# sstadick/gzp

Hardware: AMD Instinct MI355X
Metric: BGZF compress MiB/s at level 1, 550 MiB text (higher is better)
Workload: dtype u8; 1 GPU; Single MI355X: 64 KiB BGZF blocks, level 1, 550 MiB text slab, bit-exact vs libdeflate; slab_bytes=576716800, block_size=65280, blocks=8835, level=1, format=bgzf, parallelism=block-shard x1, device=AMD Radeon Graphics (gfx950:sramecc+:xnack-, 256 CUs)

## Files before the change

gzp_amd/csrc/gzpx_kernels.hip:

```cpp
#include <hip/hip_runtime.h>
#include <type_traits>
#include <cstring>

#include "gzpx_device.h"

#ifdef GZPX_EXPERIMENT
#define GZPX_EXP(cfg, bit) (((cfg).debug >> (bit)) & 1u)
#else
#define GZPX_EXP(cfg, bit) 0u
#endif

namespace gzpx {


__device__ __forceinline__ void wave_sync() {
    __builtin_amdgcn_fence(__ATOMIC_SEQ_CST, "wavefront");
    __builtin_amdgcn_wave_barrier();
    __builtin_amdgcn_fence(__ATOMIC_SEQ_CST, "wavefront");
}

__device__ __forceinline__ uint32_t rdlane(uint32_t v, uint32_t l) {
    return (uint32_t)__builtin_amdgcn_readlane((int)v, (int)l);
}
__device__ __forceinline__ uint32_t uniform(uint32_t v) { return (uint32_t)__builtin_amdgcn_readfirstlane((int)v); }

#if defined(__HIP_DEVICE_COMPILE__)
#define GZPX_PIN_VGPR(x) asm volatile("" : "+v"(x))
#else
#define GZPX_PIN_VGPR(x) ((void)0)
#endif

__device__ __forceinline__ uint32_t lz_hash15(uint32_t v) { return (v * 0x1E35A7BDu) >> 17; }

__device__ __forceinline__ uint32_t load_le32_global(const uint8_t *p) {
    const uintptr_t a = (uintptr_t)p;
    const uint32_t *w = (const uint32_t *)(a & ~(uintptr_t)3);
    return __builtin_amdgcn_alignbyte(w[1], w[0], (uint32_t)(a & 3));
}

__device__ __forceinline__ uint32_t wave_reduce_add(uint32_t v) {
    for (int m = 32; m >= 1; m >>= 1) v += __shfl_xor(v, m);
    return v;
}

__device__ __forceinline__ uint32_t wave_inclusive_scan(uint32_t v, unsigned lane) {
    for (int d = 1; d < 64; d <<= 1) {
        uint32_t t = __shfl_up(v, d);
        if (lane >= (unsigned)d) v += t;
    }
    return v;
}

template <int CTRL, int ROW_MASK>
__device__ __forceinline__ uint32_t dpp_zero(uint32_t v) {
    return (uint32_t)__builtin_amdgcn_update_dpp(0, (int)v, CTRL, ROW_MASK, 0xf, false);
}
__device__ __forceinline__ uint32_t wave_incl_add(uint32_t v) {
    v += dpp_zero<0x111, 0xf>(v);
    v += dpp_zero<0x112, 0xf>(v);
    v += dpp_zero<0x114, 0xf>(v);
    v += dpp_zero<0x118, 0xf>(v);
    v += dpp_zero<0x142, 0xa>(v);
    v += dpp_zero<0x143, 0xc>(v);
    return v;
}
__device__ __forceinline__ uint32_t umax32(uint32_t a, uint32_t b) { return a > b ? a : b; }
__device__ __forceinline__ uint32_t wave_incl_max(uint32_t v) {
    v = umax32(v, dpp_zero<0x111, 0xf>(v));
    v = umax32(v, dpp_zero<0x112, 0xf>(v));
    v = umax32(v, dpp_zero<0x114, 0xf>(v));
    v = umax32(v, dpp_zero<0x118, 0xf>(v));
    v = umax32(v, dpp_zero<0x142, 0xa>(v));
    v = umax32(v, dpp_zero<0x143, 0xc>(v));
    return v;
}

template <unsigned NW>
__device__ __forceinline__ uint32_t block_exclusive_scan(uint32_t v, uint32_t *wsum, uint32_t *total) {
    const unsigned tid = threadIdx.x, lane = tid & 63, wave = tid >> 6;
    const uint32_t inc = wave_incl_add(v);
    __syncthreads();
    if (lane == 63) wsum[wave] = inc;
    __syncthreads();
    const uint32_t mine = lane < NW ? wsum[lane] : 0u;
    const uint32_t winc = wave_incl_add(mine);
    *total = rdlane(winc, NW - 1);
    const uint32_t base = wave ? rdlane(winc, wave - 1) : 0u;
    return base + inc - v;
}

__device__ __forceinline__ uint64_t block_exclusive_scan256(uint64_t v, uint64_t *wsum, uint64_t *total) {
    const unsigned tid = threadIdx.x, lane = tid & 63, wave = tid >> 6;
    uint64_t inc = v;
    for (int d = 1; d < 64; d <<= 1) {
        const uint64_t t = __shfl_up(inc, d);
        if (lane >= (unsigned)d) inc += t;
    }
    __syncthreads();
    if (lane == 63) wsum[wave] = inc;
    __syncthreads();
    uint64_t base = 0, tot = 0;
    for (unsigned w = 0; w < 4; w++) {
        const uint64_t s = wsum[w];
        if (w < wave) base += s;
        tot += s;
    }
    *total = tot;
    return base + inc - v;
}

__device__ __forceinline__ void length_slot(uint32_t len, uint32_t &slot, uint32_t &ebits,
                                            uint32_t &eval) {
    const uint32_t x = len - 3;
    if (x < 8) {
        slot = x;
        ebits = 0;
        eval = 0;
    } else if (x == 255) {
        slot = 28;
        ebits = 0;
        eval = 0;
    } else {
        const uint32_t k = 31 - __clz((int)x);
        ebits = k - 2;
        slot = 4 * k - 4 + ((x >> ebits) & 3);
        eval = x & ((1u << ebits) - 1);
    }
}

__device__ __forceinline__ void offset_slot(uint32_t off, uint32_t &slot, uint32_t &ebits,
                                            uint32_t &eval) {
    const uint32_t d = off - 1;
    if (d < 4) {
        slot = d;
        ebits = 0;
        eval = 0;
    } else {
        const uint32_t k = 31 - __clz((int)d);
        ebits = k - 1;
        slot = 2 * k + ((d >> ebits) & 1);
        eval = d & ((1u << ebits) - 1);
    }
}


__device__ __forceinline__ uint32_t precode_order(uint32_t i) {
    const uint64_t lo = 0x22caa324e804a30ull, hi = 0x3c2e1346cull;
    return i < 12u ? (uint32_t)(lo >> (5u * i)) & 31u : (uint32_t)(hi >> (5u * (i - 12u))) & 31u;
}

__device__ __forceinline__ BlockMeta block_meta_of(const Config &cfg, uint64_t slab_len, uint32_t nb, uint32_t is_last,
                                                   uint32_t b) {
    const uint64_t begin = (uint64_t)b * cfg.block_size;
    uint64_t len = slab_len > begin ? slab_len - begin : 0;
    if (len > cfg.block_size) len = cfg.block_size;
    BlockMeta m;
    m.n = (uint32_t)len;
    m.is_last = (is_last && b == nb - 1) ? 1u : 0u;
    m.ntok = 0;
    m.nsub = 0;
    m.payload_bytes = 0;
    m.framed_bytes = 0;
    m.crc = 0;
    m.status = kStatusOk;
    return m;
}

__global__ void k_init_meta(Config cfg, uint64_t slab_len, uint32_t nb, uint32_t is_last,
                            BlockMeta *meta, uint32_t *redo) {
    const uint32_t b = blockIdx.x * blockDim.x + threadIdx.x;
    if (b == 0 && redo) {
        redo[0] = 0;
        redo[1 + nb] = 0;
    }
    if (b >= nb) return;
    meta[b] = block_meta_of(cfg, slab_len, nb, is_last, b);
}

constexpr uint32_t kBuckets = 1u << 15;
constexpr uint32_t kCandSteps = 16;

__device__ __forceinline__ uint2 cand_fetch(const uint32_t *__restrict__ in32, uint32_t mis,
                                            uint32_t p, uint32_t wmax) {
    const uint32_t w = (p + mis) >> 2;
    uint2 v;
    v.x = in32[w < wmax ? w : wmax];
    v.y = in32[w + 1 < wmax ? w + 1 : wmax];
    return v;
}

constexpr uint32_t kCandWaves = 16;

template <int MODE>
__device__ __forceinline__ bool cand_bucket(uint32_t v, uint32_t p, uint32_t &h) {
    if (MODE == 0) {
        h = p != 0 ? lz_hash15(v) : 0;
        return true;
    } else if (MODE == 1) {
        h = p != 0 ? lz_hash15(v & 0xFFFFFFu) : 0;
        return true;
    } else {
        const uint32_t h16 = p != 0 ? (v * 0x1E35A7BDu) >> 16 : 0;
        h = h16 & 32767u;
        return MODE == 2 ? h16 < 32768u : h16 >= 32768u;
    }
}

template <int MODE>
__device__ __forceinline__ void cand_step_safe(uint32_t *tab, uint32_t mis, uint32_t base,
                                               uint32_t lane, uint32_t n, uint2 raw,
                                               uint16_t *__restrict__ cand) {
    const uint32_t p = base + lane;
    uint32_t h = 0;
    const bool owns = cand_bucket<MODE>(__builtin_amdgcn_alignbyte(raw.y, raw.x, (p + mis) & 3u), p, h);
    const bool valid = owns && p + 5 <= n;
    if (!valid) h = 0;
    uint32_t c0 = tab[h];
    uint64_t same = __ballot(valid);
    for (int bit = 0; bit < 15; bit++) {
        const bool one = (h >> bit) & 1u;
        const uint64_t m = __ballot(one);
        same &= one ? m : ~m;
    }
    const uint64_t below = same & ((1ull << lane) - 1ull);
    const bool is_last_of_group = ((same >> lane) >> 1) == 0;
    if (below) c0 = (base + 63u - (uint32_t)__clzll((long long)below)) & 0xFFFFu;
    wave_sync();
    if (valid && is_last_of_group) tab[h] = p & 0xFFFFu;
    wave_sync();
    uint32_t d0 = (p - c0) & 0xFFFFu;
    if (d0 > 32767u) d0 = 0;
    if (MODE < 2 || valid || (MODE == 2 && p + 5 > n)) cand[p] = (uint16_t)(valid ? d0 : 0u);
}

template <int MODE>
__device__ void cand_block_safe(uint32_t *tab, const uint32_t *in32, uint32_t mis, uint32_t wmax, uint32_t n,
                                uint32_t lane, uint16_t *__restrict__ cand) {
    for (uint32_t i = lane; i < kBuckets; i += 64) tab[i] = 0x8000u;
    wave_sync();
    for (uint32_t base = 0; base < n; base += 64) {
        if (base != 0 && (base & 32767u) == 0) {
            const uint32_t dead = (base + 0x8000u) & 0xFFFFu;
            for (uint32_t i = lane; i < kBuckets; i += 64) {
                const uint32_t e = tab[i];
                const uint32_t a = (base - e) & 0xFFFFu;
                if (a == 0 || a > 32767u) tab[i] = dead;
            }
            wave_sync();
        }
        cand_step_safe<MODE>(tab, mis, base, lane, n, cand_fetch(in32, mis, base + lane, wmax), cand);
    }
}

template <int MODE>
__global__ __launch_bounds__(64 * kCandWaves) void k_candidates(Config cfg,
                                                                 const uint8_t *__restrict__ slab,
                                                                 BlockMeta *__restrict__ meta,
                                                                 uint16_t *__restrict__ cand_all,
                                                                 uint64_t slab_len, uint32_t nb, uint32_t is_last,
                                                                 uint32_t *__restrict__ redo, uint32_t *__restrict__ claim) {
    __shared__ uint32_t tab[kBuckets + 64];
    __shared__ uint32_t turn;
    __shared__ uint32_t bad_any;
    const uint32_t tid = threadIdx.x, lane = tid & 63u, wave = tid >> 6;
    constexpr uint32_t kIterPos = 64 * kCandSteps;
    auto block_len = [&](uint32_t blk) -> uint32_t {
        const uint64_t begin = (uint64_t)blk * cfg.block_size;
        const uint64_t len = slab_len > begin ? slab_len - begin : 0;
        return (uint32_t)(len > cfg.block_size ? cfg.block_size : len);
    };
    if (MODE <= 1) {
        for (uint32_t blk = blockIdx.x + tid * gridDim.x; blk < nb; blk += 64 * kCandWaves * gridDim.x)
            meta[blk] = block_meta_of(cfg, slab_len, nb, is_last, blk);
        if (blockIdx.x == 0 && tid == 0) redo[0] = 0;
        if (blockIdx.x == 0 && tid < 8) claim[tid] = 0;
    }
    for (uint32_t i = tid; i < kBuckets + 64; i += 64 * kCandWaves) tab[i] = 0;
    if (tid == 0) {
        turn = 0;
        bad_any = 0;
    }
    __syncthreads();

    struct Cursor {
        uint32_t b, it, n, n_iters, vbase, ibase;
    };
    auto settle = [&](Cursor &c) -> bool {
        for (;;) {
            if (c.b >= nb) return false;
            c.n = block_len(c.b);
            c.n_iters = c.n > cfg.passthrough ? (c.n + kIterPos - 1) / kIterPos : 0u;
            if (c.it < c.n_iters) return true;
            if (c.n_iters) {
                c.vbase += c.n + 32768u;
                c.ibase += c.n_iters;
// ... 2374 lines not shown
                                cl = l1;
                                co = d1;
                                continue;
                            }
                        }
                        if (lazy2) {
                            uint32_t d2 = t_d2[rr + 1u];
                            const uint32_t l2 = (uint32_t)t_l2[rr + 1u] + 3u;
                            if (d2 & kHcOrphan) d2 = cl >= 5u ? d2 & 0x7FFFu : 0u;
                            if (d2 != 0 && l2 >= cl && 4 * (int)(l2 - cl) + (bsr_cur - (31 - __clz((int)d2))) > 6) {
                                nlit += 2u;
                                cp += 2u;
                                cl = l2;
                                co = d2;
                                continue;
                            }
                        }
                        break;
                    }
                    mlen = cl;
                    moff = co;
                    nrel = cp + cl - pos;
                }
                if (mlen == 0) nrel = lane + 1u;
            }
            exp_lap(1);
            uint64_t reach = 0;
            uint32_t q = 0;
            while (q < 64u) {
                reach |= 1ull << q;
                q = (uint32_t)__builtin_amdgcn_readlane((int)nrel, (int)q);
            }
            const uint32_t exit_rel = q;
            exp_lap(2);
            const bool in_r = (reach >> lane) & 1ull;
            const uint32_t cnt = in_r ? nlit + (mlen ? 1u : 0u) : 0u;
            const uint32_t inc = wave_incl_add(cnt);
            const uint32_t tb = inc - cnt;
            const uint64_t mm = __ballot(in_r && mlen != 0);
            const uint32_t mb = (uint32_t)__popcll(mm & lane_below);
            const bool due = in_r && (p >= max_block_end || nseq + mb >= kHcSeqPerSub ||
                                      (num_new + tb >= 512u && p - sub_start >= kMinBlockLen && n - p >= kMinBlockLen) ||
                                      p >= next_recalc);
            const uint64_t dm_real = __ballot(due);
            const uint64_t dm = dm_real | (__ballot(off_tile) & reach);
            const uint32_t e = dm ? (uint32_t)__ffsll((long long)dm) - 1u : 64u;
            const uint64_t commit = e < 64u ? reach & ((1ull << e) - 1ull) : reach;
            exp_lap(3);
            if ((commit >> lane) & 1ull) {
                const uint32_t o = ti + tb;
                for (uint32_t j = 0; j < nlit; j++) {
                    const uint32_t c = t_in[r + j];
                    tok[o + j] = c;
                    atomicAdd(&L.freq[c], 1u);
                    atomicAdd(&L.nw[((c >> 5) & 6u) | (c & 1u)], 1u);
                }
                if (mlen) {
                    tok[o + nlit] = kTokMatch | (moff << 9) | mlen;
                    atomicAdd(&L.nw[8u + (mlen >= 9u ? 1u : 0u)], 1u);
                }
            }
            const uint32_t done_tok = e < 64u ? (uint32_t)__builtin_amdgcn_readlane((int)tb, (int)e)
                                              : (uint32_t)__builtin_amdgcn_readlane((int)inc, 63);
            ti += done_tok;
            num_new += done_tok;
            nseq += (uint32_t)__popcll(mm & commit);
            pos += e < 64u ? e : exit_rel;
            exp_lap(4);
            if (e == 64u) continue;
            if (!((dm_real >> e) & 1ull)) {
                t0 = 0xFFFFFFFFu;
                here = true;
                continue;
            }
            if (pos >= max_block_end || nseq >= kHcSeqPerSub) break;
            if (num_new >= 512u && pos - sub_start >= kMinBlockLen && n - pos >= kMinBlockLen) {
                __syncthreads();
                const uint32_t o = lane < 10 ? L.obs[lane] : 0u, w = lane < 10 ? L.nw[lane] : 0u;
                const uint32_t expected = o * num_new, actual = w * num_obs;
                const uint32_t total_delta = wave_reduce_add(actual > expected ? actual - expected : expected - actual);
                bool end = false;
                if (num_obs > 0) {
                    const uint32_t blen = pos - sub_start, num_items = num_obs + num_new;
                    uint32_t cutoff = num_new * 200u / 512u * num_obs;
                    if (blen < 10000u && num_items < 8192u)
                        cutoff += (uint32_t)((unsigned long long)cutoff * (8192u - num_items) / 8192u);
                    end = total_delta + (blen / 4096u) * num_obs >= cutoff;
                }
                if (end) break;
                if (lane < 10) {
                    L.obs[lane] = o + w;
                    L.nw[lane] = 0;
                }
                num_obs += num_new;
                num_new = 0;
                continue;
            }
            {
                __syncthreads();
                uint32_t f[4], total = 0;
                for (uint32_t k = 0; k < 4; k++) {
                    f[k] = L.freq[lane + 64u * k];
                    total += f[k];
                }
                total = wave_reduce_add(total);
                const uint32_t cutoff = total >> 10;
                uint32_t num_used = 0;
                for (uint32_t k = 0; k < 4; k++) num_used += (uint32_t)__popcll(__ballot(f[k] > cutoff));
                min_len = hc_choose_min_len(num_used, cfg.hc_depth);
                const uint32_t a = n - next_recalc, bb = pos - sub_start;
                next_recalc += a < bb ? a : bb;
            }
        }
        if (lane == 0) {
            sub[cur_sub].tok_begin = sub_start_tok;
            sub[cur_sub].tok_end = ti;
            sub[cur_sub].byte_begin = sub_start;
            sub[cur_sub].byte_len = pos - sub_start;
            sub[cur_sub].is_final = pos == n ? 1u : 0u;
        }
        cur_sub++;
        if (pos == n) break;
    }
    if (lane == 0) {
        meta->ntok = ti;
        meta->nsub = cur_sub;
    }
#ifdef GZPX_EXPERIMENT
    exp_lap(5);
    if (lane == 0)
        for (uint32_t k = 0; k < 8; k++) atomicAdd(&g_exp_cycles[(b & 1023u) * 8u + k], exp_acc[k]);
#endif
}

__global__ void k_hc_init(uint32_t nb, HcState *hc, uint32_t *pending) {
    const uint32_t b = blockIdx.x * blockDim.x + threadIdx.x;
    if (b == 0) *pending = 0;
    if (b >= nb) return;
    HcState s;
    s.done = 0;
    s.min_len = 0;
    s.resume_pos = 0;
    s.tok_carry = 0;
    s.mat_carry = 0;
    s.cur_sub = 0;
    s.rounds = 0;
    s.pad = 0;
    s.sparse = kHcArraysNone;
    hc[b] = s;
}

constexpr uint32_t kHistCopies = 8;
constexpr uint32_t kHistPad = kHistStride + 1;

__global__ __launch_bounds__(256) void k_hist(Config cfg, const BlockMeta *__restrict__ meta_all,
                                              const SubMeta *__restrict__ sub_all,
                                              const uint32_t *__restrict__ tok_all,
                                              uint32_t *__restrict__ hist_all) {
    __shared__ uint32_t hist[kHistCopies * kHistPad];
    const uint32_t tid = threadIdx.x;
    const uint32_t b = blockIdx.x;
    const BlockMeta *meta = meta_all + b;
    if (meta->n <= cfg.passthrough) return;
    const SubMeta *sub = sub_all + (uint64_t)b * cfg.max_sub;
    const uint32_t *tok = tok_all + (uint64_t)b * cfg.stride;
    const uint32_t nsub = meta->nsub;
    uint32_t *mine = hist + (tid & (kHistCopies - 1u)) * kHistPad;
    for (uint32_t s = 0; s < nsub; s++) {
        for (uint32_t i = tid; i < kHistCopies * kHistPad; i += 256) hist[i] = 0;
        __syncthreads();
        const uint32_t t_end = sub[s].tok_end;
        for (uint32_t t0 = sub[s].tok_begin + tid; t0 < t_end; t0 += 4 * 256) {
            uint32_t tk[4];
#pragma unroll
            for (uint32_t k = 0; k < 4; k++) tk[k] = t0 + k * 256 < t_end ? tok[t0 + k * 256] : 0xFFFFFFFFu;
#pragma unroll
            for (uint32_t k = 0; k < 4; k++) {
                const uint32_t t = tk[k];
                if (t == 0xFFFFFFFFu) continue;
                if (t & kTokMatch) {
                    uint32_t ls, le, lv, os, oe, ov;
                    length_slot(t & 0x1FFu, ls, le, lv);
                    offset_slot((t >> 9) & 0xFFFFu, os, oe, ov);
                    atomicAdd(&mine[257 + ls], 1u);
                    atomicAdd(&mine[kNumLitlen + os], 1u);
                } else {
                    atomicAdd(&mine[t], 1u);
                }
            }
        }
        __syncthreads();
        uint32_t *out = hist_all + ((uint64_t)b * cfg.max_sub + s) * kHistStride;
        for (uint32_t i = tid; i < kHistStride; i += 256) {
            uint32_t sum = 0;
#pragma unroll
            for (uint32_t c = 0; c < kHistCopies; c++) sum += hist[c * kHistPad + i];
            out[i] = sum;
        }
        __syncthreads();
    }
}

struct HuffLds {
    union {
        uint32_t key[kNumLitlen];
        uint32_t nfreq[kNumLitlen];
        uint32_t hdr[kHdrWords];
    };
    union {
        uint32_t sfreq[kNumLitlen];
        struct {
            uint32_t sfreq_low[32];
            uint16_t items[kNumLitlen + kNumOffset];
        };
    };
    union {
        uint32_t freq[kNumLitlen];
        struct {
            uint32_t freq_low[kNumLitlen / 2];
            uint16_t parent[kNumLitlen];
        };
    };
    uint32_t lcw[kNumLitlen];
    uint16_t ssym[kNumLitlen];
    uint8_t depth[kNumLitlen];
    uint8_t lens[kNumLitlen + kNumOffset];
    uint8_t olens[kNumOffset + 2];
    uint8_t plens[32];
    uint32_t ocw[kNumOffset];
    uint32_t pcw[32];
    uint32_t pfreq[32];
    uint32_t len_counts[16];
    uint32_t misc[8];
};
static_assert(sizeof(HuffLds) <= 6400, "HuffLds: 25 workgroups per CU");
static_assert(kHdrWords <= kNumLitlen, "header bits fit region A");


__device__ __forceinline__ uint32_t reg5_get(const uint32_t (&r)[5], uint32_t k) {
    const uint32_t j = k >> 6, l = k & 63u;
    uint32_t v = rdlane(r[0], l);
    const uint32_t v1 = rdlane(r[1], l), v2 = rdlane(r[2], l), v3 = rdlane(r[3], l), v4 = rdlane(r[4], l);
    v = j == 1 ? v1 : v;
    v = j == 2 ? v2 : v;
    v = j == 3 ? v3 : v;
    v = j == 4 ? v4 : v;
    return v;
}

template <uint32_t NCH, uint32_t MAXL>
__device__ void make_code(HuffLds &h, uint32_t num_syms, uint32_t compat, uint8_t *lens, uint32_t *cw, uint32_t lane) {
    constexpr uint32_t max_len = MAXL;
    uint32_t used = 0;
    for (uint32_t base = 0; base < num_syms; base += 64) {
        const uint32_t s = base + lane;
        uint32_t f = 0;
        if (s < num_syms) {
            f = h.freq[s];
            h.key[s] = f ? ((f << 10) | s) : 0xFFFFFFFFu;
            lens[s] = 0;
            cw[s] = 0;
        }
        used += (uint32_t)__popcll(__ballot(f != 0));
    }
    wave_sync();
    if (used < 2) {
        if (used == 0 && compat == 1) return;
        if (lane == 0) {
            uint32_t sym = 0;
            if (used)
                for (uint32_t s = 0; s < num_syms; s++)
                    if (h.freq[s]) sym = s;
            const uint32_t other = sym ? sym : 1;
            lens[0] = 1;
            cw[0] = 0;
            lens[other] = 1;
            cw[other] = 1;
        }
        wave_sync();
        return;
    }
    {
        uint32_t at = 0;
        uint32_t k0 = lane < num_syms ? h.key[lane] : 0xFFFFFFFFu;
        for (uint32_t base = 0; base < num_syms; base += 64) {
            const uint32_t s1 = base + 64 + lane;
            const uint32_t k1 = s1 < num_syms ? h.key[s1] : 0xFFFFFFFFu;
            wave_sync();
            const bool u = k0 != 0xFFFFFFFFu;
            const unsigned long long m = __ballot(u);
            if (u) h.key[at + (uint32_t)__popcll(m & ((1ull << lane) - 1ull))] = k0;
            at += (uint32_t)__popcll(m);
            k0 = k1;
        }
    }
    wave_sync();
    for (uint32_t base = 0; base < used; base += 64) {
        const uint32_t s = base + lane;
        const uint32_t k = s < used ? h.key[s] : 0u;
        uint32_t rank = 0;
        for (uint32_t j = 0; j < used; j++) rank += h.key[j] < k ? 1u : 0u;
        if (s < used) {
            h.sfreq[rank] = k >> 10;
            h.ssym[rank] = (uint16_t)(k & 1023u);
        }
    }
    wave_sync();
    if (lane == 0) {
        const uint32_t last = used - 1;
        uint32_t i = 0, bq = 0, e = 0;
        do {
            uint32_t nf;
            if (i + 1 <= last && (bq == e || h.sfreq[i + 1] <= h.nfreq[bq])) {
                nf = h.sfreq[i] + h.sfreq[i + 1];
                i += 2;
            } else if (bq + 2 <= e && (i > last || h.nfreq[bq + 1] < h.sfreq[i])) {
                nf = h.nfreq[bq] + h.nfreq[bq + 1];
                h.parent[bq] = (uint16_t)e;
                h.parent[bq + 1] = (uint16_t)e;
                bq += 2;
            } else {
                nf = h.sfreq[i] + h.nfreq[bq];
                h.parent[bq] = (uint16_t)e;
                i++;
                bq++;
            }
            h.nfreq[e] = nf;
        } while (++e < last);
    }
    wave_sync();
    {
        const uint32_t last = used - 1, root = last - 1;
        uint32_t par[NCH], dep[NCH];
#pragma unroll
        for (uint32_t k = 0; k < NCH; k++) {
            const uint32_t node = lane + 64 * k;
            par[k] = node < root ? h.parent[node] : 0xFFFFu;
            dep[k] = node == root ? 0u : 0xFFu;
            if (node <= root) h.depth[node] = (uint8_t)dep[k];
        }
// ... 512 lines not shown
    return total;
}

struct CrcDirectLds {
    uint32_t table[4][256];
    uint32_t part[kCrcSmall];
};

__device__ uint32_t crc32_direct(CrcDirectLds &l, const uint8_t *__restrict__ in, uint32_t n, const CrcConsts &cc,
                                 uint32_t tid) {
    constexpr uint32_t T = kCrcSmall, kSegB = 256, kChunk = T * kSegB;
    for (uint32_t i = tid; i < 256; i += T) {
        uint32_t c = i;
        for (int k = 0; k < 8; k++) c = (c >> 1) ^ (0xEDB88320u & (0u - (c & 1u)));
        l.table[0][i] = c;
    }
    __syncthreads();
    for (uint32_t i = tid; i < 256; i += T) {
        const uint32_t t0 = l.table[0][i];
        const uint32_t t1 = (t0 >> 8) ^ l.table[0][t0 & 0xFFu];
        const uint32_t t2 = (t1 >> 8) ^ l.table[0][t1 & 0xFFu];
        const uint32_t t3 = (t2 >> 8) ^ l.table[0][t2 & 0xFFu];
        l.table[1][i] = t1;
        l.table[2][i] = t2;
        l.table[3][i] = t3;
    }
    uint32_t total = 0;
    const uint32_t first_len = n ? ((n - 1) % kChunk) + 1 : 0;
    for (uint32_t cb = 0; cb < n || cb == 0; cb += (cb == 0 ? first_len : kChunk)) {
        const uint32_t clen = n == 0 ? 0 : (cb == 0 ? first_len : kChunk);
        __syncthreads();
        const int32_t seg_end_i = (int32_t)clen - (int32_t)kSegB * (int32_t)(T - 1 - tid);
        uint32_t crc = 0;
        if (seg_end_i > 0) {
            const uint32_t sb = seg_end_i > (int32_t)kSegB ? (uint32_t)seg_end_i - kSegB : 0u;
            const uint32_t len = (uint32_t)seg_end_i - sb;
            const uint8_t *p = in + cb + sb;
            uint32_t c = 0xFFFFFFFFu;
            if (len == kSegB) {
                const uint32_t mis = (uint32_t)((uintptr_t)p & 3u);
                const uint32_t *q = (const uint32_t *)(p - mis);
                const bool at_end = cb + (uint32_t)seg_end_i == n && mis == 0;
                uint32_t carry = q[0];
                for (uint32_t g = 0; g < 2; g++) {
                    dword4 v[8];
#pragma unroll
                    for (uint32_t k = 0; k < 8; k++) {
                        if (g == 1 && k == 7 && at_end) {
                            v[k].x = q[61];
                            v[k].y = q[62];
                            v[k].z = q[63];
                            v[k].w = 0;
                        } else {
                            v[k] = *(const dword4 *)(q + 1 + 32 * g + 4 * k);
                        }
                    }
#pragma unroll
                    for (uint32_t k = 0; k < 8; k++) {
                        const uint32_t w[4] = {__builtin_amdgcn_alignbyte(v[k].x, carry, mis),
                                               __builtin_amdgcn_alignbyte(v[k].y, v[k].x, mis),
                                               __builtin_amdgcn_alignbyte(v[k].z, v[k].y, mis),
                                               __builtin_amdgcn_alignbyte(v[k].w, v[k].z, mis)};
                        carry = v[k].w;
#pragma unroll
                        for (uint32_t j = 0; j < 4; j++) {
                            c ^= w[j];
                            c = l.table[3][c & 0xFFu] ^ l.table[2][(c >> 8) & 0xFFu] ^ l.table[1][(c >> 16) & 0xFFu] ^
                                l.table[0][c >> 24];
                        }
                    }
                }
            } else {
                for (uint32_t i = 0; i < len; i++) c = (c >> 8) ^ l.table[0][(c ^ p[i]) & 0xFFu];
            }
            crc = ~c;
        }
        l.part[tid] = crc;
        __syncthreads();
        for (uint32_t level = 0; level < 8; level++) {
            const uint32_t stride = 1u << level;
            const uint32_t left = 2 * stride * tid;
            uint32_t merged = 0;
            const bool act = left < T;
            if (act) merged = gf2_multmodp(cc.pow64[level + 2], l.part[left]) ^ l.part[left + stride];
            __syncthreads();
            if (act) l.part[left] = merged;
            __syncthreads();
        }
        total = cb == 0 ? l.part[0] : (gf2_multmodp(cc.pow_tile, total) ^ l.part[0]);
        if (n == 0) break;
    }
    return total;
}

__global__ __launch_bounds__(kCrcSmall) void k_crc32(Config cfg, const uint8_t *__restrict__ slab,
                                                     BlockMeta *__restrict__ meta_all, CrcConsts cc) {
    __shared__ CrcDirectLds l;
    const uint32_t b = blockIdx.x;
    const uint32_t total = crc32_direct(l, slab + (uint64_t)b * cfg.block_size, meta_all[b].n, cc, threadIdx.x);
    if (threadIdx.x == 0) meta_all[b].crc = total;
}

constexpr uint32_t kScanThreads = 1024;
__global__ __launch_bounds__(kScanThreads) void k_scan(uint32_t nb, const BlockMeta *__restrict__ meta,
                                                       uint64_t *__restrict__ out_off, uint32_t *__restrict__ sizes,
                                                       const SlabResult *__restrict__ prev,
                                                       SlabResult *__restrict__ result) {
    __shared__ uint64_t wsum[kScanThreads / 64];
    __shared__ uint32_t fail_s;
    const uint32_t tid = threadIdx.x, lane = tid & 63u, wave = tid >> 6;
    if (tid == 0) fail_s = 0xFFFFFFFFu;
    __syncthreads();
    const uint32_t per = (nb + kScanThreads - 1) / kScanThreads;
    const uint32_t i0 = tid * per < nb ? tid * per : nb, i1 = i0 + per < nb ? i0 + per : nb;
    uint64_t mine = 0;
    uint32_t bad = 0xFFFFFFFFu;
#pragma unroll 8
    for (uint32_t i = i0; i < i1; i++) {
        mine += meta[i].framed_bytes;
        if (meta[i].status != kStatusOk && bad == 0xFFFFFFFFu) bad = i;
    }
    if (bad != 0xFFFFFFFFu) atomicMin(&fail_s, bad);
    uint64_t inc = mine;
    for (int d = 1; d < 64; d <<= 1) {
        const uint64_t t = __shfl_up(inc, d);
        if (lane >= (unsigned)d) inc += t;
    }
    if (lane == 63) wsum[wave] = inc;
    __syncthreads();
    uint64_t run = prev ? prev->total : 0;
    uint64_t total = run;
    for (uint32_t w = 0; w < kScanThreads / 64; w++) {
        const uint64_t v = wsum[w];
        if (w < wave) run += v;
        total += v;
    }
    run += inc - mine;
#pragma unroll 8
    for (uint32_t i = i0; i < i1; i++) {
        const uint32_t v = meta[i].framed_bytes;
        sizes[i] = v;
        out_off[i] = run;
        run += v;
    }
    if (tid == 0) {
        const uint32_t f = fail_s;
        out_off[nb] = total;
        result->total = total;
        result->fail_block = f;
        result->fail_status = f != 0xFFFFFFFFu ? meta[f].status : kStatusOk;
    }
}

constexpr uint32_t kStageWords = 18432;

__device__ __forceinline__ void stage_or_bits(uint32_t *stage, uint32_t bitpos, uint64_t v) {
    const uint32_t w = bitpos >> 5, sh = bitpos & 31u;
    const uint64_t t = v << sh;
    const uint32_t x0 = (uint32_t)t, x1 = (uint32_t)(t >> 32);
    const uint32_t x2 = sh ? (uint32_t)(v >> (64 - sh)) : 0u;
    if (x0) atomicOr(&stage[w], x0);
    if (x1) atomicOr(&stage[w + 1], x1);
    if (x2) atomicOr(&stage[w + 2], x2);
}

__device__ __forceinline__ void stage_put_byte(uint32_t *stage, uint32_t byte_idx, uint32_t v) {
    atomicOr(&stage[byte_idx >> 2], (v & 0xFFu) << (8u * (byte_idx & 3u)));
}

constexpr uint32_t kEmitThreads = 1024;

__device__ __forceinline__ void stage_flush(const uint32_t *stage, uint8_t *dst_aligned,
                                            uint32_t win_base, uint32_t upto, uint32_t lead,
                                            uint32_t end_byte, uint32_t tid) {
    const uint32_t words = (upto - win_base + 3) >> 2;
    for (uint32_t w = tid; w < words; w += kEmitThreads) {
        const uint32_t v = stage[w];
        const uint32_t b0 = win_base + 4 * w;
        if (b0 >= lead && b0 + 4 <= end_byte && b0 + 4 <= upto) {
            *(uint32_t *)(dst_aligned + b0) = v;
        } else {
            for (uint32_t k = 0; k < 4; k++)
                if (b0 + k >= lead && b0 + k < end_byte && b0 + k < upto)
                    dst_aligned[b0 + k] = (uint8_t)(v >> (8 * k));
        }
    }
}

__device__ __forceinline__ void emit_block(const Config &cfg, const uint8_t *__restrict__ slab,
                                           const BlockMeta *__restrict__ meta_all,
                                           const SubMeta *__restrict__ sub_all,
                                           const uint32_t *__restrict__ tok_all,
                                           const uint32_t *__restrict__ codes_all,
                                           const uint32_t *__restrict__ hdr_all,
                                           const uint64_t *__restrict__ out_off,
                                           uint8_t *__restrict__ out, uint64_t out_cap, const uint32_t b,
                                           uint32_t *stage, uint32_t *codes, uint32_t *wsum, const uint8_t *lslot) {
    const uint32_t tid = threadIdx.x;
    const BlockMeta *meta = meta_all + b;
    const SubMeta *sub = sub_all + (uint64_t)b * cfg.max_sub;
    const uint32_t n = meta->n;
    const uint32_t framed = meta->framed_bytes;
    const uint32_t c = meta->payload_bytes;
    const uint64_t dst_off = out_off[b];
    if (meta->status != kStatusOk || dst_off + framed > out_cap) return;
    const uint8_t *in = slab + (uint64_t)b * cfg.block_size;
    const uint32_t hdr_len = header_bytes(cfg.format);
    const uint32_t lead = (uint32_t)(((uintptr_t)out + dst_off) & 3u);
    uint8_t *dst_aligned = out + dst_off - lead;
    const uint32_t end_byte = lead + framed;
    uint32_t win_base = 0;

    for (uint32_t i = tid; i < kStageWords; i += kEmitThreads) stage[i] = 0;
    __syncthreads();

    if (tid == 0) {
        const uint32_t hb = lead;
        stage_put_byte(stage, hb + 0, 0x1f);
        stage_put_byte(stage, hb + 1, 0x8b);
        stage_put_byte(stage, hb + 2, 8);
        stage_put_byte(stage, hb + 3, 4);
        stage_put_byte(stage, hb + 8, cfg.xfl);
        stage_put_byte(stage, hb + 9, 255);
        if (cfg.format == 0) {
            const uint32_t bsize = c + 25;
            stage_put_byte(stage, hb + 10, 6);
            stage_put_byte(stage, hb + 12, 'B');
            stage_put_byte(stage, hb + 13, 'C');
            stage_put_byte(stage, hb + 14, 2);
            stage_put_byte(stage, hb + 16, bsize);
            stage_put_byte(stage, hb + 17, bsize >> 8);
        } else {
            const uint32_t tot = c + 28;
            stage_put_byte(stage, hb + 10, 8);
            stage_put_byte(stage, hb + 12, 'I');
            stage_put_byte(stage, hb + 13, 'G');
            stage_put_byte(stage, hb + 14, 4);
            stage_put_byte(stage, hb + 16, tot);
            stage_put_byte(stage, hb + 17, tot >> 8);
            stage_put_byte(stage, hb + 18, tot >> 16);
            stage_put_byte(stage, hb + 19, tot >> 24);
        }
    }

    const uint32_t *tok = tok_all + (uint64_t)b * cfg.stride;
    const uint32_t nsub = meta->nsub;
    uint32_t bitpos = 8u * (lead + hdr_len);
    auto ensure = [&](uint32_t need_bits) {
        if (((bitpos + need_bits + 7) >> 3) + 16u <= 4u * kStageWords) return;
        __syncthreads();
        const uint32_t upto_rel = (bitpos >> 3) & ~3u;
        stage_flush(stage, dst_aligned, win_base, win_base + upto_rel, lead, end_byte, tid);
        const uint32_t keep = stage[upto_rel >> 2];
        __syncthreads();
        for (uint32_t i = tid; i < kStageWords; i += kEmitThreads) stage[i] = 0;
        __syncthreads();
        if (tid == 0) stage[0] = keep;
        win_base += upto_rel;
        bitpos -= 8u * upto_rel;
        __syncthreads();
    };
    for (uint32_t s = 0; s < nsub; s++) {
        const SubMeta sm = sub[s];
        if (sm.type == kStored) {
            uint32_t left = sm.byte_len, src = sm.byte_begin;
            do {
                const uint32_t chunk = left > 65535u ? 65535u : left;
                const bool last_chunk = chunk == left;
                ensure(64);
                if (tid == 0) stage_or_bits(stage, bitpos, (sm.is_final && last_chunk) ? 1u : 0u);
                bitpos = (bitpos + 3 + 7u) & ~7u;
                if (tid == 0) {
                    const uint32_t bytepos = bitpos >> 3;
                    stage_put_byte(stage, bytepos + 0, chunk);
                    stage_put_byte(stage, bytepos + 1, chunk >> 8);
                    stage_put_byte(stage, bytepos + 2, ~chunk);
                    stage_put_byte(stage, bytepos + 3, (~chunk) >> 8);
                }
                bitpos += 32;
                for (uint32_t done = 0; done < chunk; done += 16384u) {
                    const uint32_t piece = chunk - done < 16384u ? chunk - done : 16384u;
                    ensure(8u * piece);
                    const uint32_t bytepos = bitpos >> 3;
                    for (uint32_t i = tid; i < piece; i += kEmitThreads)
                        stage_put_byte(stage, bytepos + i, in[src + done + i]);
                    bitpos += 8u * piece;
                }
                src += chunk;
                left -= chunk;
            } while (left);
            __syncthreads();
            continue;
        }
        __syncthreads();
        const uint32_t *cd = codes_all + ((uint64_t)b * cfg.max_sub + s) * kCodeWords;
        for (uint32_t i = tid; i < kCodeWords; i += kEmitThreads) codes[i] = cd[i];
        const uint32_t *hw = hdr_all + ((uint64_t)b * cfg.max_sub + s) * kHdrWords;
        const uint32_t nhw = (sm.hdr_bits + 31) >> 5;
        ensure(32u * kHdrWords);
        for (uint32_t i = tid; i < nhw; i += kEmitThreads) stage_or_bits(stage, bitpos + 32 * i, hw[i]);
        bitpos += sm.hdr_bits;
        __syncthreads();
        const uint32_t tok_last = meta->ntok - 1;
        uint32_t tnext[4];
#pragma unroll
        for (uint32_t j = 0; j < 4; j++) {
            const uint32_t i = sm.tok_begin + 4 * tid + j;
            tnext[j] = tok[i < tok_last ? i : tok_last];
        }
        for (uint32_t tb = sm.tok_begin; tb < sm.tok_end; tb += 4 * kEmitThreads) {
            ensure(4u * kEmitThreads * 48u);
            const uint32_t t0 = tb + 4 * tid;
            uint64_t bits[4];
            uint32_t nbits[4], sum = 0;
            uint32_t tcur[4];
#pragma unroll
            for (uint32_t j = 0; j < 4; j++) tcur[j] = tnext[j];
#pragma unroll
            for (uint32_t j = 0; j < 4; j++) {
                const uint32_t i = t0 + 4 * kEmitThreads + j;
                tnext[j] = tok[i < tok_last ? i : tok_last];
            }
#pragma unroll
            for (uint32_t j = 0; j < 4; j++) {
                bits[j] = 0;
                nbits[j] = 0;
                if (t0 + j < sm.tok_end) {
                    const uint32_t t = tcur[j];
                    if (t & kTokMatch) {
                        const uint32_t len = t & 0x1FFu, off = (t >> 9) & 0xFFFFu;
                        uint32_t os, oe, ov;
                        const uint32_t lt = lslot[len - 3u];
                        const uint32_t ls = lt & 31u, le = lt >> 5, lv = (len - 3u) & ((1u << le) - 1u);
                        offset_slot(off, os, oe, ov);
                        const uint32_t lc = codes[257 + ls], oc = codes[kNumLitlen + os];
                        const uint32_t lpart = (lc & 0xFFFFu) | (lv << (lc >> 16)), lbits = (lc >> 16) + le;
                        const uint32_t opart = (oc & 0xFFFFu) | (ov << (oc >> 16)), obits = (oc >> 16) + oe;
                        bits[j] = (uint64_t)lpart | ((uint64_t)opart << lbits);
                        nbits[j] = lbits + obits;
                    } else {
                        const uint32_t lc = codes[t];
                        bits[j] = lc & 0xFFFFu;
                        nbits[j] = lc >> 16;
                    }
                    sum += nbits[j];
                }
            }
            uint32_t total;
            const uint32_t ex = block_exclusive_scan<kEmitThreads / 64>(sum, wsum, &total);
            uint32_t off_bits = bitpos + ex, accn = 0;
            uint64_t acc = 0;
#pragma unroll
            for (uint32_t j = 0; j < 4; j++) {
                if (accn + nbits[j] > 64) {
                    stage_or_bits(stage, off_bits, acc);
                    off_bits += accn;
                    acc = 0;
                    accn = 0;
                }
                acc |= bits[j] << accn;
                accn += nbits[j];
            }
            if (accn) stage_or_bits(stage, off_bits, acc);
            bitpos += total;
        }
        ensure(64);
        if (tid == 0) {
            const uint32_t ec = codes[256];
            stage_or_bits(stage, bitpos, ec & 0xFFFFu);
        }
        bitpos += codes[256] >> 16;
        __syncthreads();
    }

    ensure(8u * (8u + 28u + 8u));
    if (tid == 0) {
        const uint32_t fb = lead + hdr_len + c - win_base;
        const uint32_t crc = meta->crc;
        for (uint32_t k = 0; k < 4; k++) {
            stage_put_byte(stage, fb + k, crc >> (8 * k));
            stage_put_byte(stage, fb + 4 + k, n >> (8 * k));
        }
        if (meta->is_last && cfg.format == 0) {
            const uint8_t eof[28] = {0x1f, 0x8b, 0x08, 0x04, 0, 0, 0, 0, 0x00, 0xff, 0x06, 0x00, 0x42, 0x43,
                                     0x02, 0x00, 0x1b, 0x00, 0x03, 0x00, 0, 0, 0, 0, 0, 0, 0, 0};
            for (uint32_t k = 0; k < 28; k++) stage_put_byte(stage, fb + 8 + k, eof[k]);
        }
    }
    __syncthreads();
    stage_flush(stage, dst_aligned, win_base, end_byte, lead, end_byte, tid);
}

__global__ __launch_bounds__(kEmitThreads, 8) void k_emit(Config cfg, const uint8_t *__restrict__ slab,
                                              const BlockMeta *__restrict__ meta_all,
                                              const SubMeta *__restrict__ sub_all,
                                              const uint32_t *__restrict__ tok_all,
                                              const uint32_t *__restrict__ codes_all,
                                              const uint32_t *__restrict__ hdr_all,
                                              const uint64_t *__restrict__ out_off,
                                              uint8_t *__restrict__ out, uint64_t out_cap, uint32_t nb) {
    __shared__ uint32_t stage[kStageWords];
    __shared__ uint32_t codes[kCodeWords];
    __shared__ uint32_t wsum[kEmitThreads / 64];
    __shared__ uint8_t lslot[256];
    if (threadIdx.x < 256) {
        uint32_t ls, le, lv;
        length_slot(threadIdx.x + 3, ls, le, lv);
        lslot[threadIdx.x] = (uint8_t)(ls | (le << 5));
    }
    for (uint32_t b = blockIdx.x; b < nb; b += gridDim.x) {
        __syncthreads();
        emit_block(cfg, slab, meta_all, sub_all, tok_all, codes_all, hdr_all, out_off, out, out_cap, b, stage, codes, wsum,
                   lslot);
    }
}

struct InfLds {
    uint32_t ring_was_here;
    uint32_t lfast[1024];
    uint32_t ofast[256];
    uint32_t inr[256];
    uint32_t own[64];
    uint16_t lsorted[288];
    uint16_t osorted[32];
    uint8_t lens[320];
    uint32_t lcount[16], lfirst[16], loffs[16];
    uint32_t ocount[16], ofirst[16], ooffs[16];
};

#ifndef GZPX_INF_R
#define GZPX_INF_R 2
#endif
constexpr uint32_t kInfR = GZPX_INF_R;

enum InfKind { kInfLitlen = 0, kInfOffset = 1, kInfPrecode = 2 };

template <int KIND>
__device__ __forceinline__ uint32_t inflate_entry(uint32_t sym, uint32_t cl) {
    if (KIND == kInfPrecode) return cl | (sym << 8);
    if (KIND == kInfLitlen) {
        if (sym < 256) return cl | (sym << 8);
        if (sym == 256) return cl | (2u << 4);
        const uint32_t slot = sym - 257;
        uint32_t base, xb = 0;
        if (slot < 8) {
            base = 3 + slot;
        } else if (slot >= 28) {
            base = 258;
        } else {
            xb = (slot - 4) >> 2;
            base = 3 + ((4 + (slot & 3)) << xb);
        }
        return cl | (1u << 4) | (xb << 8) | (base << 16);
    }
    if (sym > 29) return cl | (1u << 4);
    uint32_t base, xb = 0;
    if (sym < 4) {
        base = 1 + sym;
    } else {
        xb = (sym - 2) >> 1;
        base = 1 + ((2 + (sym & 1)) << xb);
    }
    return cl | (xb << 8) | (base << 16);
}

template <int KIND>
__device__ bool inflate_build(const uint8_t *lens, uint32_t nsyms, uint32_t fast_bits, uint32_t *fast,
                              uint16_t *sorted, uint32_t *count, uint32_t *first, uint32_t *offs,
                              uint32_t lane) {
    const uint64_t lane_below = (1ull << lane) - 1ull;
    uint32_t cnt[16];
    for (uint32_t l = 0; l < 16; l++) cnt[l] = 0;
    for (uint32_t base = 0; base < nsyms; base += 64) {
        const uint32_t s = base + lane;
        const uint32_t myl = s < nsyms ? lens[s] : 0;
        for (uint32_t l = 1; l <= 15; l++) cnt[l] += (uint32_t)__popcll(__ballot(myl == l));
    }
    uint32_t code = 0, idx = 0, kraft = 0;
    uint32_t fst[16], off[16];
    for (uint32_t l = 1; l <= 15; l++) {
        code <<= 1;
        fst[l] = code;
        off[l] = idx;
        code += cnt[l];
        idx += cnt[l];
        kraft += cnt[l] << (15 - l);
    }
    if (kraft > (1u << 15)) return false;
    if (kraft < (1u << 15)) {
        if (kraft != 0 && (kraft != (1u << 14) || cnt[1] != 1)) return false;
        uint32_t only = 0;
        for (uint32_t base = 0; base < nsyms && kraft; base += 64) {
            const uint64_t m = __ballot(base + lane < nsyms && lens[base + lane] == 1);
            if (m) only = base + (uint32_t)__ffsll((long long)m) - 1;
        }
        wave_sync();
        if (lane < 16) count[lane] = 0;
        const uint32_t e = inflate_entry<KIND>(only, 1);
        for (uint32_t i = lane; i < (1u << fast_bits); i += 64) fast[i] = e;
        wave_sync();
        return true;
    }
    wave_sync();
    if (lane < 16) {
        count[lane] = lane ? cnt[lane] : 0;
        first[lane] = lane ? fst[lane] : 0;
        offs[lane] = lane ? off[lane] : 0;
    }
    for (uint32_t i = lane; i < (1u << fast_bits); i += 64) fast[i] = 0;
    wave_sync();
    uint32_t run[16];
    for (uint32_t l = 0; l < 16; l++) run[l] = 0;
    for (uint32_t base = 0; base < nsyms; base += 64) {
        const uint32_t s = base + lane;
        const uint32_t myl = s < nsyms ? lens[s] : 0;
        uint32_t rank = 0;
        for (uint32_t l = 1; l <= 15; l++) {
            const uint64_t m = __ballot(myl == l);
            if (myl == l) rank = run[l] + (uint32_t)__popcll(m & lane_below);
            run[l] += (uint32_t)__popcll(m);
        }
        if (myl) {
            sorted[off[myl] + rank] = (uint16_t)s;
            if (myl <= fast_bits) {
                const uint32_t cw = __brev(fst[myl] + rank) >> (32 - myl);
                const uint32_t e = inflate_entry<KIND>(s, myl);
                for (uint32_t k = cw; k < (1u << fast_bits); k += 1u << myl) fast[k] = e;
            }
        }
    }
    wave_sync();
    return true;
}

template <int KIND>
__device__ uint32_t inflate_slow(uint32_t bits, const uint16_t *sorted, const uint32_t *count,
                                 const uint32_t *first, const uint32_t *offs) {
    uint32_t code = 0;
    for (uint32_t l = 1; l <= 15; l++) {
        code = (code << 1) | ((bits >> (l - 1)) & 1u);
        const uint32_t c = count[l];
        if (code - first[l] < c) return inflate_entry<KIND>(sorted[offs[l] + code - first[l]], l);
    }
    return 0;
}

struct DBlock {
    uint64_t in_off;
    uint32_t size;
    uint32_t isize;
    uint32_t crc;
    uint32_t status;
    uint32_t produced;
    uint32_t nmatch;
    uint32_t pay_off;
    uint32_t pay_len;
    uint32_t cyc[8];
};

__global__ void k_dinit(uint32_t hdr_len, uint32_t nb, const uint8_t *__restrict__ in, const uint64_t *__restrict__ offsets,
                        const uint32_t *__restrict__ sizes, DBlock *__restrict__ blk, uint32_t *__restrict__ redo) {
    const uint32_t b = blockIdx.x * blockDim.x + threadIdx.x;
    if (b == 0 && redo) {
        redo[0] = 0;
        redo[1 + nb] = 0;
    }
// ... 1002 lines not shown
```

Before: 175,500 MiB/s.

## Vectorize token loads and precompute fused length codes in hist and emit kernels

The histogram and emit kernels now read tokens as 16-byte vector loads per lane with wave-uniform edge masking. They replace branchy length/offset slot computation with a branch-free offset slot and a shared table of fused length code plus extra bits. Emit packs bit counts into byte fields, so one scan sums both parts. It appends bits through a 32-bit streaming accumulator instead of 64-bit stage_or_bits calls, double-buffers the scan partials, and zeroes only the used part of the stage buffer. The risks are in the alignment assumptions of the uint4 loads, including reads past the sub-block end, and in how the null-symbol sentinel is handled.

```diff
diff --git a/gzp_amd/csrc/gzpx_kernels.hip b/gzp_amd/csrc/gzpx_kernels.hip
--- a/gzp_amd/csrc/gzpx_kernels.hip
+++ b/gzp_amd/csrc/gzpx_kernels.hip
@@ -141,6 +141,21 @@
         slot = 2 * k + ((d >> ebits) & 1);
         eval = d & ((1u << ebits) - 1);
     }
+}
+
+__device__ __forceinline__ uint32_t length_entry(uint32_t x) {
+    uint32_t ls, le, lv;
+    length_slot(x + 3, ls, le, lv);
+    return ls | (le << 5);
+}
+__device__ __forceinline__ void build_length_table(uint8_t *lslot, uint32_t tid) {
+    if (tid < 256) lslot[tid] = (uint8_t)length_entry(tid);
+}
+
+__device__ __forceinline__ void offset_slot_flat(uint32_t d, uint32_t &slot, uint32_t &ebits) {
+    const uint32_t k = 31u - (uint32_t)__clz((int)(d | 1u));
+    ebits = (uint32_t)max((int)k - 1, 0);
+    slot = 2u * k + ((d >> ebits) & 1u);
 }
 
 
@@ -2821,16 +2836,21 @@
 
 constexpr uint32_t kHistCopies = 8;
 constexpr uint32_t kHistPad = kHistStride + 1;
+constexpr uint32_t kHistStep = 2048;
+constexpr uint32_t kHistNoToken = 0x7FFFFFFFu;
+static_assert(kHistStep % 1024 == 0, "whole 16-byte loads per lane");
 
 __global__ __launch_bounds__(256) void k_hist(Config cfg, const BlockMeta *__restrict__ meta_all,
                                               const SubMeta *__restrict__ sub_all,
                                               const uint32_t *__restrict__ tok_all,
                                               uint32_t *__restrict__ hist_all) {
     __shared__ uint32_t hist[kHistCopies * kHistPad];
+    __shared__ uint8_t lslot[256];
     const uint32_t tid = threadIdx.x;
     const uint32_t b = blockIdx.x;
     const BlockMeta *meta = meta_all + b;
     if (meta->n <= cfg.passthrough) return;
+    build_length_table(lslot, tid);
     const SubMeta *sub = sub_all + (uint64_t)b * cfg.max_sub;
     const uint32_t *tok = tok_all + (uint64_t)b * cfg.stride;
     const uint32_t nsub = meta->nsub;
@@ -2838,23 +2858,36 @@
     for (uint32_t s = 0; s < nsub; s++) {
         for (uint32_t i = tid; i < kHistCopies * kHistPad; i += 256) hist[i] = 0;
         __syncthreads();
-        const uint32_t t_end = sub[s].tok_end;
-        for (uint32_t t0 = sub[s].tok_begin + tid; t0 < t_end; t0 += 4 * 256) {
-            uint32_t tk[4];
-#pragma unroll
-            for (uint32_t k = 0; k < 4; k++) tk[k] = t0 + k * 256 < t_end ? tok[t0 + k * 256] : 0xFFFFFFFFu;
-#pragma unroll
-            for (uint32_t k = 0; k < 4; k++) {
+        const uint32_t t_begin = sub[s].tok_begin, t_end = sub[s].tok_end;
+        for (uint32_t t0 = t_begin & ~3u; t0 < t_end; t0 += kHistStep) {
+            uint32_t tk[kHistStep / 256];
+#pragma unroll
+            for (uint32_t k = 0; k < kHistStep / 1024; k++) {
+                const uint4 v = *(const uint4 *)(tok + t0 + 1024u * k + 4u * tid);
+                tk[4 * k + 0] = v.x;
+                tk[4 * k + 1] = v.y;
+                tk[4 * k + 2] = v.z;
+                tk[4 * k + 3] = v.w;
+            }
+            const bool edge = t0 < t_begin || t0 + kHistStep > t_end;
+            if (edge) {
+#pragma unroll
+                for (uint32_t k = 0; k < kHistStep / 256; k++) {
+                    const uint32_t i = t0 + 1024u * (k / 4) + 4u * tid + (k & 3u);
+                    if (i < t_begin || i >= t_end) tk[k] = kHistNoToken;
+                }
+            }
+#pragma unroll
+            for (uint32_t k = 0; k < kHistStep / 256; k++) {
                 const uint32_t t = tk[k];
-                if (t == 0xFFFFFFFFu) continue;
-                if (t & kTokMatch) {
-                    uint32_t ls, le, lv, os, oe, ov;
-                    length_slot(t & 0x1FFu, ls, le, lv);
-                    offset_slot((t >> 9) & 0xFFFFu, os, oe, ov);
-                    atomicAdd(&mine[257 + ls], 1u);
+                if (edge && t == kHistNoToken) continue;
+                const bool m = (int32_t)t < 0;
+                const uint32_t lt = lslot[(t - 3u) & 0xFFu];
+                atomicAdd(&mine[m ? 257u + (lt & 31u) : t], 1u);
+                if (m) {
+                    uint32_t os, oe;
+                    offset_slot_flat(((t >> 9) & 0xFFFFu) - 1u, os, oe);
                     atomicAdd(&mine[kNumLitlen + os], 1u);
-                } else {
-                    atomicAdd(&mine[t], 1u);
                 }
             }
         }
@@ -3673,7 +3706,7 @@
     }
 }
 
-constexpr uint32_t kStageWords = 18432;
+constexpr uint32_t kStageWords = 18224;
 
 __device__ __forceinline__ void stage_or_bits(uint32_t *stage, uint32_t bitpos, uint64_t v) {
     const uint32_t w = bitpos >> 5, sh = bitpos & 31u;
@@ -3690,6 +3723,12 @@
 }
 
 constexpr uint32_t kEmitThreads = 1024;
+constexpr uint32_t kEmitTpl = 4;
+constexpr uint32_t kEmitStep = kEmitTpl * kEmitThreads;
+constexpr uint32_t kEmitLenTab = kCodeWords;
+constexpr uint32_t kEmitCodeWords = kCodeWords + 256;
+constexpr uint32_t kNullSym = 287;
+static_assert(kEmitTpl % 4 == 0 && kEmitTpl <= 8, "16-byte token loads; two byte-wide bit counts summed in one word");
 
 __device__ __forceinline__ void stage_flush(const uint32_t *stage, uint8_t *dst_aligned,
                                             uint32_t win_base, uint32_t upto, uint32_t lead,
@@ -3708,6 +3747,19 @@
     }
 }
 
+__device__ __forceinline__ uint32_t emit_scan(uint32_t v, uint32_t *wsum, uint32_t *total) {
+    constexpr unsigned NW = kEmitThreads / 64;
+    const unsigned tid = threadIdx.x, lane = tid & 63, wave = tid >> 6;
+    const uint32_t inc = wave_incl_add(v);
+    if (lane == 63) wsum[wave] = inc;
+    __syncthreads();
+    const uint32_t mine = lane < NW ? wsum[lane] : 0u;
+    const uint32_t winc = wave_incl_add(mine);
+    *total = rdlane(winc, NW - 1);
+    const uint32_t base = wave ? rdlane(winc, wave - 1) : 0u;
+    return base + inc - v;
+}
+
 __device__ __forceinline__ void emit_block(const Config &cfg, const uint8_t *__restrict__ slab,
                                            const BlockMeta *__restrict__ meta_all,
                                            const SubMeta *__restrict__ sub_all,
@@ -3716,7 +3768,7 @@
                                            const uint32_t *__restrict__ hdr_all,
                                            const uint64_t *__restrict__ out_off,
                                            uint8_t *__restrict__ out, uint64_t out_cap, const uint32_t b,
-                                           uint32_t *stage, uint32_t *codes, uint32_t *wsum, const uint8_t *lslot) {
+                                           uint32_t *stage, uint32_t *codes, uint32_t *wsum) {
     const uint32_t tid = threadIdx.x;
     const BlockMeta *meta = meta_all + b;
     const SubMeta *sub = sub_all + (uint64_t)b * cfg.max_sub;
@@ -3732,7 +3784,8 @@
     const uint32_t end_byte = lead + framed;
     uint32_t win_base = 0;
 
-    for (uint32_t i = tid; i < kStageWords; i += kEmitThreads) stage[i] = 0;
+    const uint32_t used_words = (end_byte + 3) >> 2 < kStageWords ? (end_byte + 3) >> 2 : kStageWords;
+    for (uint32_t i = tid; i < used_words; i += kEmitThreads) stage[i] = 0;
     __syncthreads();
 
     if (tid == 0) {
@@ -3815,82 +3868,106 @@
         }
         __syncthreads();
         const uint32_t *cd = codes_all + ((uint64_t)b * cfg.max_sub + s) * kCodeWords;
-        for (uint32_t i = tid; i < kCodeWords; i += kEmitThreads) codes[i] = cd[i];
+        if (tid < kEmitCodeWords) {
+            uint32_t e;
+            if (tid < kNumLitlen) {
+                const uint32_t lc = cd[tid];
+                e = tid == kNullSym ? 0u : (lc & 0xFFFFu) | (lc >> 16 << 24);
+            } else if (tid < kEmitLenTab) {
+                e = cd[tid];
+            } else {
+                const uint32_t x = tid - kEmitLenTab, lt = length_entry(x);
+                const uint32_t lc = cd[257u + (lt & 31u)], le = lt >> 5;
+                e = (lc & 0xFFFFu) | ((x & ((1u << le) - 1u)) << (lc >> 16)) | (((lc >> 16) + le) << 24);
+            }
+            codes[tid] = e;
+        }
         const uint32_t *hw = hdr_all + ((uint64_t)b * cfg.max_sub + s) * kHdrWords;
         const uint32_t nhw = (sm.hdr_bits + 31) >> 5;
         ensure(32u * kHdrWords);
         for (uint32_t i = tid; i < nhw; i += kEmitThreads) stage_or_bits(stage, bitpos + 32 * i, hw[i]);
         bitpos += sm.hdr_bits;
         __syncthreads();
-        const uint32_t tok_last = meta->ntok - 1;
-        uint32_t tnext[4];
-#pragma unroll
-        for (uint32_t j = 0; j < 4; j++) {
-            const uint32_t i = sm.tok_begin + 4 * tid + j;
-            tnext[j] = tok[i < tok_last ? i : tok_last];
-        }
-        for (uint32_t tb = sm.tok_begin; tb < sm.tok_end; tb += 4 * kEmitThreads) {
-            ensure(4u * kEmitThreads * 48u);
-            const uint32_t t0 = tb + 4 * tid;
-            uint64_t bits[4];
-            uint32_t nbits[4], sum = 0;
-            uint32_t tcur[4];
-#pragma unroll
-            for (uint32_t j = 0; j < 4; j++) tcur[j] = tnext[j];
-#pragma unroll
-            for (uint32_t j = 0; j < 4; j++) {
-                const uint32_t i = t0 + 4 * kEmitThreads + j;
-                tnext[j] = tok[i < tok_last ? i : tok_last];
-            }
-#pragma unroll
-            for (uint32_t j = 0; j < 4; j++) {
-                bits[j] = 0;
-                nbits[j] = 0;
-                if (t0 + j < sm.tok_end) {
-                    const uint32_t t = tcur[j];
-                    if (t & kTokMatch) {
-                        const uint32_t len = t & 0x1FFu, off = (t >> 9) & 0xFFFFu;
-                        uint32_t os, oe, ov;
-                        const uint32_t lt = lslot[len - 3u];
-                        const uint32_t ls = lt & 31u, le = lt >> 5, lv = (len - 3u) & ((1u << le) - 1u);
-                        offset_slot(off, os, oe, ov);
-                        const uint32_t lc = codes[257 + ls], oc = codes[kNumLitlen + os];
-                        const uint32_t lpart = (lc & 0xFFFFu) | (lv << (lc >> 16)), lbits = (lc >> 16) + le;
-                        const uint32_t opart = (oc & 0xFFFFu) | (ov << (oc >> 16)), obits = (oc >> 16) + oe;
-                        bits[j] = (uint64_t)lpart | ((uint64_t)opart << lbits);
-                        nbits[j] = lbits + obits;
-                    } else {
-                        const uint32_t lc = codes[t];
-                        bits[j] = lc & 0xFFFFu;
-                        nbits[j] = lc >> 16;
+        const uint32_t wtok = uniform((tid >> 6) * (64u * kEmitTpl));
+        const uint32_t *ltok = tok + kEmitTpl * tid;
+        uint4 tnext[kEmitTpl / 4];
+        if ((sm.tok_begin & ~3u) + wtok < sm.tok_end) {
+#pragma unroll
+            for (uint32_t q = 0; q < kEmitTpl / 4; q++) tnext[q] = *(const uint4 *)(ltok + (sm.tok_begin & ~3u) + 4 * q);
+        }
+        uint32_t step = 0;
+        for (uint32_t tb = sm.tok_begin & ~3u; tb < sm.tok_end; tb += kEmitStep) {
+            uint32_t pa[kEmitTpl], pb[kEmitTpl], nn[kEmitTpl], sumnn = 0;
+#pragma unroll
+            for (uint32_t j = 0; j < kEmitTpl; j++) pa[j] = pb[j] = nn[j] = 0;
+            const bool live = tb + wtok < sm.tok_end;
+            if (live) {
+                uint32_t t[kEmitTpl];
+#pragma unroll
+                for (uint32_t q = 0; q < kEmitTpl / 4; q++) {
+                    t[4 * q + 0] = tnext[q].x;
+                    t[4 * q + 1] = tnext[q].y;
+                    t[4 * q + 2] = tnext[q].z;
+                    t[4 * q + 3] = tnext[q].w;
+                }
+                if (tb + wtok < sm.tok_begin || tb + wtok + 64u * kEmitTpl > sm.tok_end) {
+#pragma unroll
+                    for (uint32_t j = 0; j < kEmitTpl; j++) {
+                        const uint32_t i = tb + kEmitTpl * tid + j;
+                        if (i < sm.tok_begin || i >= sm.tok_end) t[j] = kNullSym;
                     }
-                    sum += nbits[j];
+                }
+#pragma unroll
+                for (uint32_t j = 0; j < kEmitTpl; j++) {
+                    const uint32_t tk = t[j];
+                    const bool m = (int32_t)tk < 0;
+                    const uint32_t lc = codes[m ? kEmitLenTab + ((tk - 3u) & 0xFFu) : tk];
+                    const uint32_t d = m ? ((tk >> 9) & 0xFFFFu) - 1u : 0u;
+                    uint32_t os, oe;
+                    offset_slot_flat(d, os, oe);
+                    const uint32_t oc = codes[kNumLitlen + os] & (uint32_t)((int32_t)tk >> 31);
+                    pa[j] = lc & 0xFFFFFFu;
+                    pb[j] = (oc & 0xFFFFu) | ((d & ((1u << oe) - 1u)) << (oc >> 16));
+                    nn[j] = (lc >> 24) | (((oc >> 16) + oe) << 8);
+                    sumnn += nn[j];
+                }
+                if (tb + kEmitStep + wtok < sm.tok_end) {
+#pragma unroll
+                    for (uint32_t q = 0; q < kEmitTpl / 4; q++) tnext[q] = *(const uint4 *)(ltok + tb + kEmitStep + 4 * q);
                 }
             }
             uint32_t total;
-            const uint32_t ex = block_exclusive_scan<kEmitThreads / 64>(sum, wsum, &total);
-            uint32_t off_bits = bitpos + ex, accn = 0;
-            uint64_t acc = 0;
-#pragma unroll
-            for (uint32_t j = 0; j < 4; j++) {
-                if (accn + nbits[j] > 64) {
-                    stage_or_bits(stage, off_bits, acc);
-                    off_bits += accn;
-                    acc = 0;
-                    accn = 0;
-                }
-                acc |= bits[j] << accn;
-                accn += nbits[j];
-            }
-            if (accn) stage_or_bits(stage, off_bits, acc);
+            const uint32_t ex = emit_scan((sumnn & 0xFFu) + (sumnn >> 8), wsum + (kEmitThreads / 64) * (step & 1u), &total);
+            step++;
+            ensure(total);
+            if (live) {
+                uint32_t *w = stage + ((bitpos + ex) >> 5);
+                uint32_t accn = (bitpos + ex) & 31u, lo = 0;
+                auto append = [&](uint32_t v, uint32_t nbits) {
+                    lo |= v << accn;
+                    accn += nbits;
+                    if (accn >= 32u) {
+                        atomicOr(w, lo);
+                        w++;
+                        accn -= 32u;
+                        lo = v >> (nbits - accn);
+                    }
+                };
+#pragma unroll
+                for (uint32_t j = 0; j < kEmitTpl; j++) {
+                    append(pa[j], nn[j] & 0xFFu);
+                    append(pb[j], nn[j] >> 8);
+                }
+                if (lo) atomicOr(w, lo);
+            }
             bitpos += total;
         }
         ensure(64);
         if (tid == 0) {
             const uint32_t ec = codes[256];
-            stage_or_bits(stage, bitpos, ec & 0xFFFFu);
-        }
-        bitpos += codes[256] >> 16;
+            stage_or_bits(stage, bitpos, ec & 0xFFFFFFu);
+        }
+        bitpos += codes[256] >> 24;
         __syncthreads();
     }
 
@@ -3921,18 +3998,11 @@
                                               const uint64_t *__restrict__ out_off,
                                               uint8_t *__restrict__ out, uint64_t out_cap, uint32_t nb) {
     __shared__ uint32_t stage[kStageWords];
-    __shared__ uint32_t codes[kCodeWords];
-    __shared__ uint32_t wsum[kEmitThreads / 64];
-    __shared__ uint8_t lslot[256];
-    if (threadIdx.x < 256) {
-        uint32_t ls, le, lv;
-        length_slot(threadIdx.x + 3, ls, le, lv);
-        lslot[threadIdx.x] = (uint8_t)(ls | (le << 5));
-    }
+    __shared__ uint32_t codes[kEmitCodeWords];
+    __shared__ uint32_t wsum[2 * (kEmitThreads / 64)];
     for (uint32_t b = blockIdx.x; b < nb; b += gridDim.x) {
         __syncthreads();
-        emit_block(cfg, slab, meta_all, sub_all, tok_all, codes_all, hdr_all, out_off, out, out_cap, b, stage, codes, wsum,
-                   lslot);
+        emit_block(cfg, slab, meta_all, sub_all, tok_all, codes_all, hdr_all, out_off, out, out_cap, b, stage, codes, wsum);
     }
 }
 
```

Result: faster. 179,000 MiB/s (median of 6 runs) (+2.0%).
